# probabilists/zuko

Measured on AMD Instinct MI355X. Metric: log_prob samples/sec, NSF d=64 K=8 bins=8 batch=2^20, higher is better.
Workload: dtype f32; 1 GPU; NSF(features=64, context=0, transforms=8, bins=8, hidden=[256]*3) log_prob, batch=2^20 per GPU, x~N(0,1), seed-0 init; batch_per_gpu=1048576, global_batch=1048576, parallelism=batch-sharded x1, one RCCL all-reduce of the scalar NLL

## Files before the change

### zuko_amd/csrc/fused_ar_half_impl.h

```cpp
#pragma once
#include "fused_ar_split_impl.h"

#ifndef ARH_LOOK
#define ARH_LOOK 1
#endif
#ifndef ARH_RELU_INT
#define ARH_RELU_INT 0
#endif

namespace zk {

typedef _Float16 f16x8 __attribute__((ext_vector_type(8)));

struct ArhB {
  f16x8 h, l;
};

__device__ __forceinline__ void arh_scale(float amax, float& s, float& inv_s) {
  amax = fmaxf(amax, __shfl_xor(amax, 16, 64));
  amax = fmaxf(amax, __shfl_xor(amax, 32, 64));
  int e = __builtin_amdgcn_frexp_expf(amax);
  int ea = 15 - e;
  ea = ea > 90 ? 90 : (ea < -90 ? -90 : ea);
  s = __builtin_amdgcn_ldexpf(1.0f, ea);
  inv_s = __builtin_amdgcn_ldexpf(1.0f, -ea);
}

__device__ __forceinline__ void arh_split(const f32x4& lo, const f32x4& hi, float s, ArhB& b) {
  if (ARX_ABL == 6) {
    b.h = __builtin_bit_cast(f16x8, lo); b.l = __builtin_bit_cast(f16x8, hi);
    return;
  }
#pragma unroll
  for (int e = 0; e < 8; ++e) {
    const float v = (e < 4 ? lo[e] : hi[e - 4]) * s;
    const _Float16 h = (_Float16)v;
    const float r = v - (float)h;
    b.h[e] = h;
    b.l[e] = (_Float16)r;
  }
}

#define ARH_MFMA(A, B, C) C = __builtin_amdgcn_mfma_f32_16x16x32_f16(__builtin_bit_cast(f16x8, A), B, C, 0, 0, 0)
__device__ __forceinline__ void arh_block(const f32x4 (&a)[2], const ArhB& b, f32x4& c) {
  if (ARX_ABL == 2) {
    asm volatile("" ::"v"(a[0]), "v"(a[1]));
    return;
  }
  ARH_MFMA(a[1], b.h, c);
  ARH_MFMA(a[0], b.l, c);
  ARH_MFMA(a[0], b.h, c);
}

__device__ __forceinline__ void arh_touch(f32x4& v) { asm volatile("" : "+v"(v)); }
template <int N> __device__ __forceinline__ void arh_settle(f32x4& a0, f32x4& a1) { asm volatile("s_waitcnt lgkmcnt(%2)" : "+v"(a0), "+v"(a1) : "n"(N)); }
template <int N> __device__ __forceinline__ void arh_settle(f32x4& a0, f32x4& a1, f32x4& a2) { asm volatile("s_waitcnt lgkmcnt(%3)" : "+v"(a0), "+v"(a1), "+v"(a2) : "n"(N)); }

template <class S, int L, class Ring> __device__ __forceinline__ void arh_hidden(Ring& ring, const float* bias_q, const ArhB (&in)[S::TMAX / 2], f32x4 (&out)[S::TMAX], float d) {
  typedef ArxPat<S> P;
  constexpr int NB = S::NB[L], BASE = S::BASE[L], HTL = S::HT[L];
  ars_for<HTL>([&](auto t_) ARS_ALWAYS_INLINE {
    constexpr int t = t_;
    if constexpr (!P::tile_has_blocks(L, t)) out[t] = *reinterpret_cast<const f32x4*>(bias_q + t * 16);
  });
  if constexpr (NB > 0) {
    constexpr int LOOK = ARH_LOOK < NB ? ARH_LOOK : NB;
    f32x4 a[LOOK + 1][2];
    f32x4 bs;
    f32x4 acc;
    const unsigned bias_addr = arx_lds_addr(bias_q);
    ars_for<LOOK>([&](auto b_) ARS_ALWAYS_INLINE {
      constexpr int b = b_;
      ars_for<2>([&](auto p) ARS_ALWAYS_INLINE { a[b][p] = ring.template read<BASE + 2 * b + decltype(p)::value>(); });
    });
    ars_for<NB>([&](auto s_) ARS_ALWAYS_INLINE {
      constexpr int s = s_, ot = P::ot(L, s), ip = P::ip(L, s), cur = s % (LOOK + 1);
      constexpr bool first_of_tile = (s == 0 || P::ot(L, s - 1) != ot), last_of_tile = (s + 1 == NB || P::ot(L, s + 1) != ot);
      if constexpr (first_of_tile) acc = f32x4{0.f, 0.f, 0.f, 0.f};
      if constexpr (last_of_tile) bs = arx_lds_raw<ot * 64>(bias_addr);
      if constexpr (s + LOOK < NB) {
        constexpr int nx = (s + LOOK) % (LOOK + 1);
        ars_for<2>([&](auto p) ARS_ALWAYS_INLINE { a[nx][p] = ring.template read<BASE + 2 * (s + LOOK) + decltype(p)::value>(); });
      }
      constexpr int ahead = (s + LOOK < NB ? LOOK : NB - 1 - s);
      if constexpr (last_of_tile) arh_settle<(s + LOOK < NB ? 2 : 0)>(a[cur][0], a[cur][1], bs);
      else arh_settle<2 * ahead>(a[cur][0], a[cur][1]);
      if (ARX_FENCE) __builtin_amdgcn_sched_barrier(0);
      arh_block(a[cur], in[ip], acc);
      if (ARX_FENCE) __builtin_amdgcn_sched_barrier(0);
      if constexpr (last_of_tile) {
#pragma unroll
        for (int r = 0; r < 4; ++r) out[ot][r] = __builtin_fmaf(acc[r], d, bs[r]);
      }
    });
  }
}

template <class S, int L, class Ring> __device__ __forceinline__ void arh_hidden_stack(Ring& ring, const float* bias_lds, int q, ArhB (&in)[S::TMAX / 2], f32x4 (&out)[S::TMAX], const ArArgs& a,
                                                                                       float& inv_s) {
  if constexpr (L < S::NH) {
    arh_hidden<S, L>(ring, bias_lds + L * S::BIAS_STRIDE + 4 * q, in, out, a.wdescale[L] * inv_s);
    constexpr int HTL = S::HT[L];
    float amax = 0.f;
    if constexpr (S::ACT == 1) {
#pragma unroll
      for (int t = 0; t < HTL; ++t)
#pragma unroll
        for (int r = 0; r < 4; ++r) {
          if (ARH_RELU_INT) out[t][r] = __builtin_bit_cast(float, max(__builtin_bit_cast(int, out[t][r]), 0));
          else out[t][r] = out[t][r] < 0.f ? 0.f : out[t][r];
          amax = fmaxf(amax, out[t][r]);
        }
    } else {
      if constexpr (S::ACT != 0) {
#pragma unroll 1
        for (int rep = 0; rep < 1; ++rep) {
#pragma unroll
          for (int t = 0; t < HTL; ++t)
#pragma unroll
            for (int r = 0; r < 4; ++r) out[t][r] = act_f32(out[t][r], S::ACT);
        }
      }
#pragma unroll
      for (int t = 0; t < HTL; ++t)
#pragma unroll
        for (int r = 0; r < 4; ++r) amax = fmaxf(amax, fabsf(out[t][r]));
    }
    float s;
    arh_scale(amax, s, inv_s);
    const f32x4 zero = {0.f, 0.f, 0.f, 0.f};
#pragma unroll
    for (int p = 0; p < (HTL + 1) / 2; ++p) arh_split(out[2 * p], 2 * p + 1 < HTL ? out[2 * p + 1] : zero, s, in[p]);
    arh_hidden_stack<S, L + 1, Ring>(ring, bias_lds, q, in, out, a, inv_s);
  }
}

template <class S, typename Uni, bool DIAG = false> __global__ __launch_bounds__(64 * S::WAVES, S::OCC) void arh_kernel(ArArgs a) {
  typedef ArRingS<S::WAVES, S::CH, S::NR> Ring;
  static_assert(S::WAVES == 8 && S::NR == 3 && S::TMAX <= 16 && S::TMAX % 2 == 0 && S::OCC == 2, "two-part split kernels: widths <= 256, two wavefronts per SIMD");
  constexpr int NT = Uni::NT, FPL = Uni::FPL, TOTAL = Uni::TOTAL, WAVES = S::WAVES;
  constexpr int NG = S::NG;
  constexpr int NSTEP = S::GOFF[NG];
  constexpr bool XLDS = S::XLDS;
  constexpr bool FID_REGS = NG * FPL <= 32;
  constexpr int DT = (S::D + 15) / 16;
  const int tid = threadIdx.x;
  const int lane = tid & 63;
  const int wave = __builtin_amdgcn_readfirstlane(tid >> 6);
  const int j = lane & 15, q = lane >> 4;

  Ring ring;
  float* bias_lds = ars_lds + S::NR * S::CH * AR_TF;
  ring.lds = ars_lds; ring.stream = a.stream; ring.n_chunks = a.n_chunks; ring.wave = wave; ring.lane = lane;
  ring.load_chunk = 0; ring.load_slot = 0;
#pragma unroll
  for (int i = 0; i < S::NR - 1; ++i) ring.issue();
  ring.slot = S::NR - 1;
  ring.lds_off = (unsigned)(size_t)((__attribute__((address_space(3))) float*)ars_lds);
  ring.cur_off = ring.lds_off;

  for (int i = tid; i < a.bias_floats; i += 64 * WAVES) bias_lds[i] = a.bias[i];
  int* fmap_lds = reinterpret_cast<int*>(bias_lds + a.bias_floats);
  float* xr = reinterpret_cast<float*>(fmap_lds + 1024 + 256) + wave * 16 * a.xs + j * a.xs;
  for (int i = tid; i < NG * 4 * FPL; i += 64 * WAVES) fmap_lds[i] = a.featmap[i];
  __syncthreads();
  const float* bias_last = bias_lds + S::NH * S::BIAS_STRIDE;
  const unsigned bias_last_addr = arx_lds_addr(bias_last + 4 * q);
  int fids[FID_REGS ? NG * FPL : 1];
  if constexpr (FID_REGS) {
#pragma unroll
    for (int i = 0; i < NG; ++i)
#pragma unroll
      for (int fi = 0; fi < FPL; ++fi) fids[i * FPL + fi] = fmap_lds[(i * 4 + q) * FPL + fi];
  }

  for (int64_t tile = blockIdx.x; tile < a.n_tiles; tile += gridDim.x) {
    const int64_t n = tile * (16 * WAVES) + wave * 16 + j;
    const bool live = n < a.N;
    const int64_t nc = live ? n : a.N - 1;
    const float* xrow = a.x + nc * a.ldx;

    ArhB in[S::TMAX / 2];
    f32x4 out[S::TMAX];
    float poison = 0.f;
    float inv_s;
    {
      f32x4 xin[S::NIT + 1];
#pragma unroll
      for (int it = 0; it < S::NIT; ++it) {
        f32x4 v = {0.f, 0.f, 0.f, 0.f};
        if ((it + 1) * 16 <= S::DIN || it * 16 + 4 * q < S::DIN) v = *reinterpret_cast<const f32x4*>(xrow + it * 16 + 4 * q);
        xin[it] = v;
      }
      xin[S::NIT] = f32x4{0.f, 0.f, 0.f, 0.f};
      int bad = 0;
      float amax = 0.f;
#pragma unroll
      for (int it = 0; it < S::NIT; ++it)
#pragma unroll
        for (int r = 0; r < 4; ++r) {
          bad |= !(fabsf(xin[it][r]) < __builtin_inff());
          amax = fmaxf(amax, fabsf(xin[it][r]));
        }
      bad |= __shfl_xor(bad, 16, 64);
      bad |= __shfl_xor(bad, 32, 64);
      if (bad) poison = __builtin_nanf("");
      if constexpr (XLDS) {
#pragma unroll
        for (int it = 0; it < DT; ++it)
          if ((it + 1) * 16 <= S::D || it * 16 + 4 * q < S::D) *reinterpret_cast<f32x4*>(xr + it * 16 + 4 * q) = xin[it];
        asm volatile("" ::: "memory");
        __builtin_amdgcn_wave_barrier();
      }
      float s;
      arh_scale(amax, s, inv_s);
#pragma unroll
      for (int p = 0; p < (S::NIT + 1) / 2; ++p) arh_split(xin[2 * p], xin[2 * p + 1], s, in[p]);
    }

    arh_hidden_stack<S, 0, Ring>(ring, bias_lds, q, in, out, a, inv_s);

    const float dl = a.wdescale[S::NH] * inv_s;
    float lacc = 0.f;
    constexpr int NBL = NSTEP * NT;
    constexpr int LOOKL = ARH_LOOK < NBL ? ARH_LOOK : NBL;
    f32x4 w[LOOKL + 1][2];
    ars_for<LOOKL>([&](auto b_) ARS_ALWAYS_INLINE {
      constexpr int b = b_;
      ars_for<2>([&](auto p) ARS_ALWAYS_INLINE { w[b][p] = ring.template read<S::LAST_BASE + 2 * b + decltype(p)::value>(); });
    });
    ars_for<NG>([&](auto g_) ARS_ALWAYS_INLINE {
      constexpr int g = g_, ST0 = S::GOFF[g], GN = S::GOFF[g + 1] - S::GOFF[g];
      int fid[FPL];
      float xin[FPL];
#pragma unroll
      for (int fi = 0; fi < FPL; ++fi) {
        if constexpr (FID_REGS) fid[fi] = fids[g * FPL + fi];
        else fid[fi] = fmap_lds[(g * 4 + q) * FPL + fi];
        const int fc = fid[fi] < 0 ? 0 : fid[fi];
        if constexpr (XLDS) xin[fi] = xr[fc];
        else xin[fi] = xrow[fc];
      }
      f32x4 acc[NT], bs[NT];
      if constexpr (GN == 0) {
        const float* bg = bias_last + (g * NT) * 16 + 4 * q;
        ars_for<NT>([&](auto t) ARS_ALWAYS_INLINE { bs[t] = *reinterpret_cast<const f32x4*>(bg + t * 16); });
      }
      ars_for<NT>([&](auto t) ARS_ALWAYS_INLINE { acc[t] = f32x4{0.f, 0.f, 0.f, 0.f}; });
      ars_for<GN>([&](auto i_) ARS_ALWAYS_INLINE {
        constexpr int st = ST0 + decltype(i_)::value, ip = S::G_IP[st];
        ars_for<NT>([&](auto t_) ARS_ALWAYS_INLINE {
          constexpr int t = t_, blk = st * NT + t, cur = blk % (LOOKL + 1);
          constexpr bool last_of_group = (decltype(i_)::value == GN - 1 && t == NT - 1);
          if constexpr (last_of_group) {
            ars_for<NT>([&](auto u) ARS_ALWAYS_INLINE { bs[u] = arx_lds_raw<(g * NT + decltype(u)::value) * 64>(bias_last_addr); });
          }
          if constexpr (blk + LOOKL < NBL) {
            constexpr int nx = (blk + LOOKL) % (LOOKL + 1);
            ars_for<2>([&](auto p) ARS_ALWAYS_INLINE { w[nx][p] = ring.template read<S::LAST_BASE + 2 * (blk + LOOKL) + decltype(p)::value>(); });
          }
          constexpr int ahead = (blk + LOOKL < NBL ? LOOKL : NBL - 1 - blk);
          if constexpr (last_of_group) arh_settle<(blk + LOOKL < NBL ? 2 : 0)>(w[cur][0], w[cur][1]);
          else arh_settle<2 * ahead>(w[cur][0], w[cur][1]);
          if constexpr (last_of_group) {
#pragma unroll
            for (int u = 0; u < NT; ++u) arh_touch(bs[u]);
          }
          if (ARX_FENCE) __builtin_amdgcn_sched_barrier(0);
          arh_block(w[cur], in[ip], acc[t]);
          if (ARX_FENCE) __builtin_amdgcn_sched_barrier(0);
        });
      });
      float p[4 * NT];
      ars_for<NT>([&](auto t) ARS_ALWAYS_INLINE {
#pragma unroll
        for (int r = 0; r < 4; ++r) p[4 * t + r] = __builtin_fmaf(acc[t][r], dl, bs[t][r]);
      });
#pragma unroll
      for (int fi = 0; fi < FPL; ++fi) Uni::template poison<false>(p, fi * TOTAL, poison);
      auto ld = [&](int i) { return p[i]; };
#pragma unroll
      for (int fi = 0; fi < FPL; ++fi) {
        const int f = fid[fi];
        if (f >= 0) {
          float yv, lj;
          if (ARX_ABL == 3) {
            yv = p[fi * TOTAL] + xin[fi]; lj = p[fi * TOTAL + 1];
#pragma unroll
            for (int i = 2; i < TOTAL; ++i) lj += p[fi * TOTAL + i];
          } else if constexpr (DIAG) {
            int kb = 0;
            float ks[Uni::NKNOT];
            Uni::fwd(ld, fi * TOTAL, a, xin[fi], yv, lj, &kb, ks);
            if (live) {
              a.bin_out[n * S::D + f] = kb;
#pragma unroll
              for (int jj = 0; jj < Uni::NKNOT; ++jj) a.knots_out[(n * S::D + f) * Uni::NKNOT + jj] = ks[jj];
            }
          } else
          Uni::fwd(ld, fi * TOTAL, a, xin[fi], yv, lj);
          if constexpr (XLDS) xr[f] = yv;
          else if (live) a.y[n * a.ldy + f] = yv;
          lacc += lj;
        }
      }
    });
    if constexpr (XLDS) {
      asm volatile("" ::: "memory");
      __builtin_amdgcn_wave_barrier();
      if (live) {
#pragma unroll
        for (int it = 0; it < DT; ++it)
          if ((it + 1) * 16 <= S::D || it * 16 + 4 * q < S::D) *reinterpret_cast<f32x4*>(a.y + n * a.ldy + it * 16 + 4 * q) = *reinterpret_cast<const f32x4*>(xr + it * 16 + 4 * q);
      }
    }
    if (a.ladj) {
      lacc += __shfl_xor(lacc, 16, 64);
      lacc += __shfl_xor(lacc, 32, 64);
      if (live && q == 0) a.ladj[n] = a.accumulate ? a.ladj[n] + lacc : lacc;
    }
  }
  asm volatile("s_waitcnt vmcnt(0)" ::: "memory");
}

template <class S, typename Uni> static int arh_launch(const ArArgs* in, int abi, int args_bytes, int train, void* stream) {
  if (abi != ARS_ABI || args_bytes != (int)sizeof(ArArgs)) return ZK_EINVAL;
  ArArgs a = *in;
  if (train || a.D != S::D || a.DIN != S::DIN || a.L != S::NH + 1 || a.act != S::ACT || a.sched || a.NG != S::NG || a.n_chunks != S::NCHUNK || a.l1rev) return ZK_EINVAL;
  for (int l = 0; l <= S::NH; ++l)
    if (!(a.wdescale[l] > 0.f) || !(a.wdescale[l] < __builtin_inff())) return ZK_EINVAL;
  a.n_tiles = (a.N + 16 * S::WAVES - 1) / (16 * S::WAVES);
  a.xs = ((S::D + 3) / 4) * 4 + 4;
  const bool vec_ok = (S::D % 4 == 0) && (a.ldy % 4 == 0) && ((uintptr_t)a.y % 16 == 0);
  if (S::XLDS != 0 && !vec_ok) return ZK_EINVAL;
  a.xlds = S::XLDS;
  const int lds = (S::NR * S::CH * AR_TF + a.bias_floats + 1024 + 256 + (S::XLDS ? S::WAVES * 16 * a.xs : 0)) * (int)sizeof(float);
  if (lds > 160 * 1024) return ZK_EINVAL;
  const void* fn = nullptr;
  if ((a.bin_out != nullptr) != (a.knots_out != nullptr)) return ZK_EINVAL;
  if (a.bin_out) {
    if constexpr (Uni::NKNOT > 1) fn = (const void*)arh_kernel<S, Uni, true>;
  } else {
    fn = (const void*)arh_kernel<S, Uni, false>;
  }
  if (!fn) return ZK_EINVAL;
  hipError_t e = hipSuccess;
  {
    static std::mutex mu;
    static std::unordered_map<const void*, int> granted;
    std::lock_guard<std::mutex> lock(mu);
    int& g = granted[fn];
    if (g < lds) {
      e = hipFuncSetAttribute(fn, hipFuncAttributeMaxDynamicSharedMemorySize, lds);
// ... 13 lines not shown
```

### zuko_amd/static_ar.py

```python

from __future__ import annotations

import ctypes
import fcntl
import hashlib
import json
import math
import os
import shutil
import subprocess
import sys
import threading

import numpy as np

HERE = os.path.dirname(os.path.abspath(__file__))
CSRC = os.path.join(HERE, "csrc")
ARS_DIR = os.path.join(HERE, "lib", "ars")
ARS_ABI = 9
UNI_TYPES = {0: "zk::UniAffine", 1: "zk::UniRqs8", 2: "zk::UniRqs4", 3: "zk::UniRqs16", 4: "zk::UniCircRqs8", 5: "zk::UniSos3x5", 6: "zk::UniBern17"}
SPLIT_ONLY_KINDS = {3, 5, 6}
_HEADERS = ("fused_ar_static_impl.h", "fused_ar_split_impl.h", "zk_ar_common.h", "zk_univariate.h", "zk_univariate_bwd.h", "zk_common.h", "zk_half.h")


# ... 244 lines not shown
        GOFFP.append(len(G_IP))
    last_base = cursor
    cursor += 3 * len(blocks)
    n_chunks = -(-cursor // ch)
    pad_blocks = -(-(n_chunks * ch - cursor) // 3)
    blocks_of.append(blocks + [-np.ones((64, 8), dtype=np.int64)] * pad_blocks)
    stream_images = max(n_chunks * ch, cursor + 3 * pad_blocks)
    gathers = [np.stack(b).astype(np.int32).reshape(-1) if b else np.zeros(0, np.int32) for b in blocks_of]
    out = dict(t)
    for key in ("S_OTG", "S_IT", "S_MASK", "NS", "GOFF", "G_IT"):
        out.pop(key)
    nr = 2 if ch == 48 else 3
    per_cu = 2 if (waves == 4 and not wide) else 1
    xlds = int(t["D"] % 4 == 0 and (nr * ch * 256 + (t["BIAS_STRIDE"] * NH + t["NG"] * nt * 16) + 1024 + 256 + waves * 16 * (((t["D"] + 3) // 4) * 4 + 4)) * 4 * per_cu <= 160 * 1024)
    out.update({"split": 1, "TMAX": int(2 * -(-t["TMAX"] // 2)), "NB": NB, "B_OT": B_OT, "B_IP": B_IP, "BASE": BASE, "LAST_BASE": last_base, "GOFF": GOFFP, "G_IP": G_IP, "NCHUNK": n_chunks, "STREAM_IMAGES": stream_images,
                "WAVES": waves, "CH": ch, "NR": nr, "XLDS": xlds, "OCC": 1 if wide else 2})
    plan._split_cache = ((uni_kind, act, split_geometry()), (out, gathers))
    return out, gathers


def half_enabled() -> bool:
    from . import fused

    return split_enabled() and fused.matmul_precision() == "f16x2"


def half_tables(plan, uni_kind: int, act: int = 1):
    ts = split_tables(plan, uni_kind, act)
    if ts is None:
        return None
    t, gathers = ts
    if t["WAVES"] != 8 or t["NH"] > 3 or uni_kind in SPLIT_ONLY_KINDS or t["CH"] != 24:
        return None
    cached = getattr(plan, "_half_cache", None)
    if cached is not None and cached[0] == (uni_kind, act):
        return cached[1]
    ch, NH, nt = t["CH"], t["NH"], plan.layout.nt
    n_last = t["GOFF"][-1] * nt
    cursor = 2 * (sum(t["NB"]) + n_last)
    n_chunks = -(-cursor // ch)
    pad_blocks = -(-(n_chunks * ch - cursor) // 2)
    last = gathers[NH][: n_last * 512]
    g = [np.asarray(x) for x in gathers[:NH]] + [np.concatenate([last, -np.ones(pad_blocks * 512, dtype=np.int32)]).astype(np.int32)]
    out = {k: v for k, v in t.items() if k not in ("split", "TRAIN_OK")}
    out.update({"half": 1, "BASE": [2 * sum(t["NB"][:l]) for l in range(NH)], "LAST_BASE": 2 * sum(t["NB"]), "NCHUNK": n_chunks, "STREAM_IMAGES": max(n_chunks * ch, cursor + 2 * pad_blocks),
                "NR": 3, "TRAIN_OK": 0})
    plan._half_cache = ((uni_kind, act), (out, g))
    return out, g


def emit_half(t: dict) -> str:
    boff = [0]
    for n in t["NB"]:
        boff.append(boff[-1] + n)
    lines = [
        "// generated by zuko_amd/static_ar.py — do not edit",
        '#include "fused_ar_half_impl.h"',
        "namespace {",
        "struct Shape {",
        f"  static constexpr int D = {t['D']}, DIN = {t['DIN']}, NIT = {t['NIT']}, NH = {t['NH']}, TMAX = {t['TMAX']}, NG = {t['NG']}, NCHUNK = {t['NCHUNK']};",
        f"  static constexpr int BIAS_STRIDE = {t['BIAS_STRIDE']}, LAST_BASE = {t['LAST_BASE']}, WAVES = {t['WAVES']}, CH = {t['CH']}, NR = {t['NR']}, ACT = {t['ACT']}, OCC = {t['OCC']};",
        f"  static constexpr bool XLDS = {'true' if t['XLDS'] else 'false'};",
        _arr("HT", "int", t["HT"]), _arr("NB", "int", t["NB"]), _arr("BOFF", "int", boff), _arr("BASE", "int", t["BASE"]),
        _arr("B_OT", "unsigned char", t["B_OT"]), _arr("B_IP", "unsigned char", t["B_IP"]), _arr("GOFF", "int", t["GOFF"]), _arr("G_IP", "unsigned char", t["G_IP"]),
        "};",
        "}  // namespace",
        f'extern "C" int zk_ars_launch(const zk::ArArgs* a, int abi, int args_bytes, int train, void* stream) {{ return zk::arh_launch<Shape, {UNI_TYPES[t["uni"]]}>(a, abi, args_bytes, train, stream); }}',
        "",
    ]
    return "\n".join(lines)


def compile_half(t: dict, verbose: bool = False, out_dir: str | None = None) -> dict | None:
    stamp = _half_digest()
    sig = _digest({"half": t, "headers": stamp})
    meta = {"so": f"arh_{sig}.so", "core": "h" + _digest(t), "half": 1, "split": 2, "l0": [], "alt": None, "headers": stamp, "uni": t["uni"], "ACT": t["ACT"], "D": t["D"], "DIN": t["DIN"], "HT": t["HT"],
            "WAVES": t["WAVES"], "CH": t["CH"], "TRAIN_OK": 0, "XLDS": t["XLDS"], "NCHUNK": t["NCHUNK"]}
    so = _build_so(f"arh_{sig}", lambda: emit_half(t), meta, verbose, out_dir)
    if so is None:
        return None
    global _INDEX
# ... 539 lines not shown
                    cands.append(chain_tables_for(lins, full=True, packed={"uni": layout.kind, "featmap": pl.featmap, "nt": layout.nt, "fpl": layout.fpl, "total": layout.total}))
                for tg in cands:
                    if tg is not None and not any(c[0] == tg[0] for c in chains):
                        chains.append(tg)
        for pl in (pa, pd):
            ts = split_tables(pl, layout.kind, act)
            if ts is not None and not any(x == ts[0] for x in splits):
                splits.append(ts[0])
            th = half_tables(pl, layout.kind, act)
            if th is not None and not any(x == th[0] for x in halves):
                halves.append(th[0])
        if layout.kind in SPLIT_ONLY_KINDS:
            continue
        ta, td = tables(pa, layout.kind, act), tables(pd, layout.kind, act)
        if ta is None or td is None:
            raise RuntimeError(f"zuko_amd.static_ar: no static kernel for the prebuilt shape {entry}")
        (ca, la), (cdesc, ld) = _split(ta), _split(td)
        if ca == cdesc:
            work.append((ta, None if la == ld else ld))
        else:
            work += [(ta, None), (td, None)]
    prev = os.environ.get("ZUKO_AMD_SPLIT_GEOM")
    if prev is None:
        os.environ["ZUKO_AMD_SPLIT_GEOM"] = "4x16"
        try:
            kind, features, context, hidden, bins = PREBUILT[0][:5]
            for pl, layout, _ in _plans_for(kind, features, context, hidden, bins):
                pl._split_cache = None
                ts = split_tables(pl, layout.kind, 1)
                if ts is not None and not any(x == ts[0] for x in splits):
                    splits.append(ts[0])
        finally:
            del os.environ["ZUKO_AMD_SPLIT_GEOM"]
    with ThreadPoolExecutor(max_workers=jobs) as ex:
        metas = list(ex.map(lambda w: compile_kernel(w[0], w[1], verbose, ARS_DIR), work))
        kerns = list(ex.map(lambda tg: chain_kernel(tg[0], True, verbose, ARS_DIR), chains))
        xmetas = list(ex.map(lambda t: compile_split(t, verbose, ARS_DIR), splits))
        hmetas = list(ex.map(lambda t: compile_half(t, verbose, ARS_DIR), halves))
    if any(m is None for m in metas + xmetas + hmetas) or any(k is None for k in kerns):
        raise RuntimeError("zuko_amd.static_ar: a prebuilt static kernel failed to compile")
    return [m["so"] for m in metas + xmetas + hmetas] + [os.path.basename(k.so) for k in kerns]


if __name__ == "__main__":
    sys.path.insert(0, os.path.dirname(HERE))
    import zuko_amd.static_ar as me

    print("\n".join(me.prebuild()))
```

### zuko_amd/csrc/zk_ar_common.h

```cpp
#pragma once
#include "zk_univariate.h"

namespace zk {

typedef float f32x4 __attribute__((ext_vector_type(4)));

#define AR_TF 256
#define AR_WAVES 8
#define AR_T 16
#define ARS_ABI 9

struct ArArgs {
  int64_t N;
  int D, DIN;
  const float* x; int64_t ldx;
  float* y; int64_t ldy;
  const float* yin; int64_t ldyin;
  float* ladj; int accumulate;
  const float* stream;
  const float* bias;
  const uint32_t* skip;
  const int32_t* featmap;
  int L, NG, n_chunks, act, bias_floats, dbg;
  const int* sched;
  int n_sched;
  int olim[8];
  int g0, g1;
  int xlds;
  int xs;
  float bound, ls;
  RqsLeanConst lc;
  int64_t n_tiles;
  int32_t* bin_out;
  float* knots_out;
  int l1rev;
  float* act_out[3];
  float* phi_out;
  int64_t ldphi;
  const float* gate[3];
  const float* phi_in;
  float* gphi_out;
  int64_t ldpin;
  const float* gy; int64_t ldgy;
// ... 13 lines not shown
    case 4: return v / (1.f + expf(-v));
    case 5: return 0.5f * v * (1.f + erff(v * 0.70710678118654752440f));
    case 6: return 1.f / (1.f + expf(-v));
    case 7: return v > 0.f ? v : 0.01f * v;
    default: return v;
  }
}


struct UniAffine {
  static constexpr int TOTAL = 2, FPL = 2, NT = 1;
  template <bool INV> static __device__ __forceinline__ void poison(float* p, int base, float nan_or_zero) {
    p[base + 0] += nan_or_zero;
    p[base + 1] += nan_or_zero;
  }
  static constexpr int NKNOT = 1;
  template <typename P, typename A> static __device__ __forceinline__ void fwd(const P& p, int base, const A& a, float x, float& y, float& lj, int* k = nullptr, float* ks = nullptr) {
    affine_fwd<float, MathFast>(p(base + 0), p(base + 1), a.ls, x, y, lj);
  }
  template <typename P, typename A> static __device__ __forceinline__ float inv(const P& p, int base, const A& a, float y) {
    return affine_inv<float, MathFast>(p(base + 0), p(base + 1), a.ls, y);
  }
};

template <int K, bool CIRC> struct UniRqs {
  static constexpr int TOTAL = 3 * K - 1, FPL = 1, NT = (TOTAL + 3) / 4;
  static __device__ __forceinline__ float shift(float v, float bound) {
    const float period = 2.f * bound;
    float r = fmodf(v, period);
    r = (r < 0.f) ? r + period : r;
    return r - bound;
  }
  template <bool INV> static __device__ __forceinline__ void poison(float* p, int base, float nan_or_zero) {
#pragma unroll
    for (int j = 0; j < K; ++j) p[base + (INV ? K : 0) + j] += nan_or_zero;
  }
  static constexpr int NKNOT = K + 1;
  template <typename P, typename A> static __device__ __forceinline__ void fwd(const P& p, int base, const A& a, float x, float& y, float& lj, int* k = nullptr, float* ks = nullptr) {
    int kk;
    rqs_lean<K, false>([&](int j) { return p(base + j); }, [&](int j) { return p(base + K + j); }, [&](int j) { return p(base + 2 * K + j); }, a.lc,
                       CIRC ? shift(x, a.bound) : x, y, lj, kk, ks);
    if (k) *k = kk;
  }
  template <typename P, typename A> static __device__ __forceinline__ float inv(const P& p, int base, const A& a, float y) {
    float x, lj;
    rqs_lean<K, true>([&](int j) { return p(base + j); }, [&](int j) { return p(base + K + j); }, [&](int j) { return p(base + 2 * K + j); }, a.lc, y, x, lj);
    return CIRC ? shift(x, a.bound) : x;
  }
};
template <int P, int L1> struct UniSos {
  static constexpr int TOTAL = P * L1 + 1, FPL = 1, NT = (TOTAL + 3) / 4, NKNOT = 1;
  template <bool INV> static __device__ __forceinline__ void poison(float* p, int base, float nan_or_zero) {
    p[base] += nan_or_zero;
    p[base + P * L1] += nan_or_zero;
  }
  template <typename Pa, typename A> static __device__ __forceinline__ void fwd(const Pa& p, int base, const A& a, float x, float& y, float& lj, int* k = nullptr, float* ks = nullptr) {
    auto ld = [&](int j) { return p(base + j); };
    y = sos_f_static<float, P, L1>(a.sos, ld, x) + p(base + P * L1);
    lj = t_log(sos_g_static<float, P, L1>(a.sos, ld, x));
  }
};
template <int NC> struct UniBernBounded {
  static constexpr int TOTAL = NC - 5, FPL = 1, NT = (TOTAL + 3) / 4, NKNOT = 1;
  template <bool INV> static __device__ __forceinline__ void poison(float* p, int base, float nan_or_zero) { p[base] += nan_or_zero; }
  template <typename Pa, typename A> static __device__ __forceinline__ void fwd(const Pa& p, int base, const A& a, float x, float& y, float& lj, int* k = nullptr, float* ks = nullptr) {
    float th[NC];
    bern_theta_bounded<float, NC>([&](int j) { return p(base + j); }, a.bound, th);
    const BernTails<float> t = bern_tails<float, NC>(th, true, a.bound, a.eps);
// ... 14 lines not shown
```

### zuko_amd/fused.py

```python

from __future__ import annotations

from dataclasses import dataclass

import ctypes
import math
import os

import numpy as np
import torch
from torch import Tensor

TILE = 16
CHUNK = 24
GROUP_HIDDEN = 4
MAX_WIDTH = 256
MAX_WIDTH_WIDE = 512


@dataclass
class UniLayout:

    kind: int
    total: int
# ... 336 lines not shown
_precision = None


def matmul_precision() -> str:
    global _precision
    if _precision is None:
        _precision = _PRECISIONS.get(os.environ.get("ZUKO_AMD_MATMUL", "f16x2").lower(), "f16x2")
    return _precision


def set_matmul_precision(mode: str) -> None:
    global _precision
    if mode.lower() not in _PRECISIONS:
        raise ValueError(f"zuko_amd.set_matmul_precision: unknown mode '{mode}' (one of {sorted(_PRECISIONS)})")
    _precision = _PRECISIONS[mode.lower()]


HALF_SPREAD_LOG2 = 14
HALF_SMALL_FRACTION = 0.01
HALF_ROW_LOG2 = 12
HALF_MIN_LOG2, HALF_MAX_LOG2 = -20, 40


def half_scales(linears):
    stats = []
    for m in linears:
        w = m.weight.detach()
        a = (w * m.mask).abs() if getattr(m, "mask", None) is not None else w.abs()
        big = a.amax()
        nz = a > 0
        small = (nz & (a < big * 2.0 ** -HALF_SPREAD_LOG2)).sum() / nz.sum().clamp_min(1)
        rowmax = a.amax(dim=1)
        minrow = torch.where(rowmax > 0, rowmax, big).amin()
        stats.append(torch.stack([big.float(), small.float(), minrow.float()]))
    out = []
    for big, small, minrow in torch.stack(stats).tolist():
        if big == 0.0:
            out.append((True, 0))
            continue
        ok = math.isfinite(big) and 2.0 ** HALF_MIN_LOG2 <= big <= 2.0 ** HALF_MAX_LOG2 and small <= HALF_SMALL_FRACTION and minrow >= big * 2.0 ** -HALF_ROW_LOG2
        out.append((bool(ok), 15 - math.frexp(big)[1] if math.isfinite(big) else 0))
    return out


def chunk_of(variant: int = 0) -> int:
    return CHUNK


def default_variant() -> int:
    return 0


class FusedAR:

    def __init__(self, plan: ArPlan, device: torch.device, act: int, bound: float, slope: float, variant: int = 0) -> None:
        self.plan = plan
        self.variant = variant
        self.device = device
        self.act = act
        self.bound = bound
        self.slope = slope
        self.skip = torch.from_numpy(plan.skip.view(np.int32).copy()).to(device)
        self.featmap = torch.from_numpy(plan.featmap.copy()).to(device)
        self.gather = [torch.from_numpy(g).to(device) for g in plan.gather]
        self.bias_gather = [torch.from_numpy(g).to(device) for g in plan.bias_gather]
        self.stream = torch.empty(plan.n_blocks * 256, dtype=torch.float32, device=device)
        self.bias_floats = plan.bias_off[-1] + len(plan.bias_gather[-1])
        self.bias = torch.empty(self.bias_floats, dtype=torch.float32, device=device)
        self._stamp = None
        self._fine_stamp = None
        self.generic_ok = plan.max_width <= MAX_WIDTH and plan.layout.kind <= 4
        self.eps = 1e-6
        self._gl = None
# ... 280 lines not shown
```

Before: 70.82 million samples/s.

## Use fma_mix f16 split, asm ReLU, packed descale, and selectable half ring geometry

```diff
diff --git a/zuko_amd/csrc/fused_ar_half_impl.h b/zuko_amd/csrc/fused_ar_half_impl.h
--- a/zuko_amd/csrc/fused_ar_half_impl.h
+++ b/zuko_amd/csrc/fused_ar_half_impl.h
@@ -26,19 +26,123 @@
   inv_s = __builtin_amdgcn_ldexpf(1.0f, -ea);
 }
 
+#ifndef ARH_SPLIT_FORM
+#define ARH_SPLIT_FORM 4
+#endif
+typedef _Float16 f16x2 __attribute__((ext_vector_type(2)));
+typedef float f32x2 __attribute__((ext_vector_type(2)));
+
 __device__ __forceinline__ void arh_split(const f32x4& lo, const f32x4& hi, float s, ArhB& b) {
   if (ARX_ABL == 6) {
     b.h = __builtin_bit_cast(f16x8, lo); b.l = __builtin_bit_cast(f16x8, hi);
     return;
   }
-#pragma unroll
-  for (int e = 0; e < 8; ++e) {
-    const float v = (e < 4 ? lo[e] : hi[e - 4]) * s;
-    const _Float16 h = (_Float16)v;
-    const float r = v - (float)h;
-    b.h[e] = h;
-    b.l[e] = (_Float16)r;
-  }
+  if constexpr (ARH_SPLIT_FORM == 0) {
+#pragma unroll
+    for (int e = 0; e < 8; ++e) {
+      const float v = (e < 4 ? lo[e] : hi[e - 4]) * s;
+      const _Float16 h = (_Float16)v;
+      const float r = v - (float)h;
+      b.h[e] = h;
+      b.l[e] = (_Float16)r;
+    }
+  } else {
+    typedef unsigned u32x4 __attribute__((ext_vector_type(4)));
+    u32x4 hp, lp;
+#pragma unroll
+    for (int p = 0; p < 4; ++p) {
+      const float x0 = p < 2 ? lo[2 * p] : hi[2 * p - 4], x1 = p < 2 ? lo[2 * p + 1] : hi[2 * p - 3];
+      if constexpr (ARH_SPLIT_FORM == 1) {
+        const f32x2 v = f32x2{x0, x1} * f32x2{s, s};
+        const f16x2 h = __builtin_convertvector(v, f16x2);
+        const f32x2 r = v - __builtin_convertvector(h, f32x2);
+        hp[p] = __builtin_bit_cast(unsigned, h);
+        lp[p] = __builtin_bit_cast(unsigned, __builtin_convertvector(r, f16x2));
+      } else if constexpr (ARH_SPLIT_FORM == 2) {
+        const float v0 = x0 * s, v1 = x1 * s;
+        const f16x2 h = __builtin_convertvector(f32x2{v0, v1}, f16x2);
+        const float r0 = v0 - (float)h[0], r1 = v1 - (float)h[1];
+        hp[p] = __builtin_bit_cast(unsigned, h);
+        lp[p] = __builtin_bit_cast(unsigned, __builtin_convertvector(f32x2{r0, r1}, f16x2));
+      } else if constexpr (ARH_SPLIT_FORM == 3) {
+        const float v0 = x0 * s, v1 = x1 * s;
+        unsigned h, l;
+        asm("v_cvt_pk_f16_f32 %0, %1, %2" : "=v"(h) : "v"(v0), "v"(v1));
+        asm("v_fma_mixlo_f16 %0, %1, 1.0, -%2 op_sel_hi:[0,0,1]" : "=v"(l) : "v"(v0), "v"(h));
+        asm("v_fma_mixhi_f16 %0, %1, 1.0, -%2 op_sel:[0,0,1] op_sel_hi:[0,0,1]" : "+v"(l) : "v"(v1), "v"(h));
+        hp[p] = h;
+        lp[p] = l;
+      } else {
+        unsigned h, l;
+        asm("v_fma_mixlo_f16 %0, %1, %2, 0" : "=v"(h) : "v"(x0), "v"(s));
+        asm("v_fma_mixhi_f16 %0, %1, %2, 0" : "+v"(h) : "v"(x1), "v"(s));
+        asm("v_fma_mixlo_f16 %0, %1, %2, -%3 op_sel_hi:[0,0,1]" : "=v"(l) : "v"(x0), "v"(s), "v"(h));
+        asm("v_fma_mixhi_f16 %0, %1, %2, -%3 op_sel:[0,0,1] op_sel_hi:[0,0,1]" : "+v"(l) : "v"(x1), "v"(s), "v"(h));
+        hp[p] = h;
+        lp[p] = l;
+      }
+    }
+    b.h = __builtin_bit_cast(f16x8, hp);
+    b.l = __builtin_bit_cast(f16x8, lp);
+  }
+}
+
+#ifndef ARH_RELU_FORM
+#define ARH_RELU_FORM 1
+#endif
+__device__ __forceinline__ void arh_relu(f32x4& v) {
+  if constexpr (ARH_RELU_FORM == 0) {
+#pragma unroll
+    for (int r = 0; r < 4; ++r) v[r] = v[r] < 0.f ? 0.f : v[r];
+  } else if constexpr (ARH_RELU_FORM == 2) {
+#pragma unroll
+    for (int r = 0; r < 4; ++r) {
+      float x = v[r];
+      asm("v_max_f32 %0, 0, %0" : "+v"(x));
+      v[r] = x;
+    }
+  } else if constexpr (ARH_RELU_FORM == 3) {
+#pragma unroll
+    for (int r = 0; r < 4; ++r) {
+      float x = v[r];
+      int t;
+      asm("v_add_i32 %1, %0, %2 clamp\n\t"
+          "v_ashrrev_i32 %1, 31, %1\n\t"
+          "v_bfi_b32 %0, %1, 0, %0"
+          : "+v"(x), "=&v"(t) : "s"(0x7fffff));
+      v[r] = x;
+    }
+  } else {
+    unsigned long long m0, m1, m2, m3;
+    float a = v[0], b = v[1], c = v[2], d = v[3];
+    asm("s_nop 0\n\t"
+        "v_cmp_ngt_f32_e64 %4, 0, %0\n\t"
+        "v_cmp_ngt_f32_e64 %5, 0, %1\n\t"
+        "v_cmp_ngt_f32_e64 %6, 0, %2\n\t"
+        "v_cmp_ngt_f32_e64 %7, 0, %3\n\t"
+        "v_cndmask_b32_e64 %0, 0, %0, %4\n\t"
+        "v_cndmask_b32_e64 %1, 0, %1, %5\n\t"
+        "v_cndmask_b32_e64 %2, 0, %2, %6\n\t"
+        "v_cndmask_b32_e64 %3, 0, %3, %7"
+        : "+v"(a), "+v"(b), "+v"(c), "+v"(d), "=&s"(m0), "=&s"(m1), "=&s"(m2), "=&s"(m3));
+    v = f32x4{a, b, c, d};
+  }
+}
+
+#ifndef ARH_DESCALE_PK
+#define ARH_DESCALE_PK 1
+#endif
+__device__ __forceinline__ f32x4 arh_descale(const f32x4& acc, float d, const f32x4& bs) {
+  f32x4 o;
+  if constexpr (ARH_DESCALE_PK) {
+    const f32x2 dd = {d, d};
+    const f32x2 lo = __builtin_elementwise_fma(f32x2{acc[0], acc[1]}, dd, f32x2{bs[0], bs[1]}), hi = __builtin_elementwise_fma(f32x2{acc[2], acc[3]}, dd, f32x2{bs[2], bs[3]});
+    o = f32x4{lo[0], lo[1], hi[0], hi[1]};
+  } else {
+#pragma unroll
+    for (int r = 0; r < 4; ++r) o[r] = __builtin_fmaf(acc[r], d, bs[r]);
+  }
+  return o;
 }
 
 #define ARH_MFMA(A, B, C) C = __builtin_amdgcn_mfma_f32_16x16x32_f16(__builtin_bit_cast(f16x8, A), B, C, 0, 0, 0)
@@ -88,10 +192,7 @@
       if (ARX_FENCE) __builtin_amdgcn_sched_barrier(0);
       arh_block(a[cur], in[ip], acc);
       if (ARX_FENCE) __builtin_amdgcn_sched_barrier(0);
-      if constexpr (last_of_tile) {
-#pragma unroll
-        for (int r = 0; r < 4; ++r) out[ot][r] = __builtin_fmaf(acc[r], d, bs[r]);
-      }
+      if constexpr (last_of_tile) out[ot] = arh_descale(acc, d, bs);
     });
   }
 }
@@ -104,13 +205,16 @@
     float amax = 0.f;
     if constexpr (S::ACT == 1) {
 #pragma unroll
-      for (int t = 0; t < HTL; ++t)
-#pragma unroll
-        for (int r = 0; r < 4; ++r) {
-          if (ARH_RELU_INT) out[t][r] = __builtin_bit_cast(float, max(__builtin_bit_cast(int, out[t][r]), 0));
-          else out[t][r] = out[t][r] < 0.f ? 0.f : out[t][r];
-          amax = fmaxf(amax, out[t][r]);
+      for (int t = 0; t < HTL; ++t) {
+        if (ARH_RELU_INT) {
+#pragma unroll
+          for (int r = 0; r < 4; ++r) out[t][r] = __builtin_bit_cast(float, max(__builtin_bit_cast(int, out[t][r]), 0));
+        } else {
+          arh_relu(out[t]);
         }
+#pragma unroll
+        for (int r = 0; r < 4; ++r) amax = fmaxf(amax, out[t][r]);
+      }
     } else {
       if constexpr (S::ACT != 0) {
 #pragma unroll 1
@@ -137,7 +241,7 @@
 
 template <class S, typename Uni, bool DIAG = false> __global__ __launch_bounds__(64 * S::WAVES, S::OCC) void arh_kernel(ArArgs a) {
   typedef ArRingS<S::WAVES, S::CH, S::NR> Ring;
-  static_assert(S::WAVES == 8 && S::NR == 3 && S::TMAX <= 16 && S::TMAX % 2 == 0 && S::OCC == 2, "two-part split kernels: widths <= 256, two wavefronts per SIMD");
+  static_assert(S::WAVES == 8 && (S::NR == 2 || S::NR == 3) && S::TMAX <= 16 && S::TMAX % 2 == 0 && S::OCC == 2, "two-part split kernels: widths <= 256, two wavefronts per SIMD");
   constexpr int NT = Uni::NT, FPL = Uni::FPL, TOTAL = Uni::TOTAL, WAVES = S::WAVES;
   constexpr int NG = S::NG;
   constexpr int NSTEP = S::GOFF[NG];
diff --git a/zuko_amd/static_ar.py b/zuko_amd/static_ar.py
--- a/zuko_amd/static_ar.py
+++ b/zuko_amd/static_ar.py
@@ -300,10 +300,11 @@
     t, gathers = ts
     if t["WAVES"] != 8 or t["NH"] > 3 or uni_kind in SPLIT_ONLY_KINDS or t["CH"] != 24:
         return None
+    geom = half_geometry(t, plan.bias_off[-1] + len(plan.bias_gather[-1]))
     cached = getattr(plan, "_half_cache", None)
-    if cached is not None and cached[0] == (uni_kind, act):
+    if cached is not None and cached[0] == (uni_kind, act, geom):
         return cached[1]
-    ch, NH, nt = t["CH"], t["NH"], plan.layout.nt
+    (ch, nr), NH, nt = geom, t["NH"], plan.layout.nt
     n_last = t["GOFF"][-1] * nt
     cursor = 2 * (sum(t["NB"]) + n_last)
     n_chunks = -(-cursor // ch)
@@ -312,9 +313,35 @@
     g = [np.asarray(x) for x in gathers[:NH]] + [np.concatenate([last, -np.ones(pad_blocks * 512, dtype=np.int32)]).astype(np.int32)]
     out = {k: v for k, v in t.items() if k not in ("split", "TRAIN_OK")}
     out.update({"half": 1, "BASE": [2 * sum(t["NB"][:l]) for l in range(NH)], "LAST_BASE": 2 * sum(t["NB"]), "NCHUNK": n_chunks, "STREAM_IMAGES": max(n_chunks * ch, cursor + 2 * pad_blocks),
-                "NR": 3, "TRAIN_OK": 0})
-    plan._half_cache = ((uni_kind, act), (out, g))
+                "CH": ch, "NR": nr, "TRAIN_OK": 0})
+    plan._half_cache = ((uni_kind, act, geom), (out, g))
     return out, g
+
+
+HALF_GEOMS = ((24, 3), (32, 3), (48, 2))
+HALF_GEOM_PREFERENCE = ((24, 3),)
+LDS_BYTES = 160 * 1024
+
+
+def half_lds_bytes(t: dict, bias_floats: int, ch: int, nr: int) -> int:
+    xs = ((t["D"] + 3) // 4) * 4 + 4
+    return (nr * ch * 256 + bias_floats + 1024 + 256 + (t["WAVES"] * 16 * xs if t["XLDS"] else 0)) * 4
+
+
+def half_geometry(t: dict, bias_floats: int) -> tuple:
+    env = os.environ.get("ZUKO_AMD_HALF_GEOM")
+    cands = HALF_GEOM_PREFERENCE
+    if env:
+        try:
+            c, n = (int(v) for v in env.split("x"))
+            if (c, n) in HALF_GEOMS:
+                cands = ((c, n),)
+        except ValueError:
+            pass
+    for c, n in cands:
+        if half_lds_bytes(t, bias_floats, c, n) <= LDS_BYTES:
+            return (c, n)
+    return (24, 3)
 
 
 def emit_half(t: dict) -> str:
@@ -920,6 +947,18 @@
                     splits.append(ts[0])
         finally:
             del os.environ["ZUKO_AMD_SPLIT_GEOM"]
+    prev = os.environ.get("ZUKO_AMD_HALF_GEOM")
+    if prev is None:
+        try:
+            for ch, nr in HALF_GEOMS:
+                os.environ["ZUKO_AMD_HALF_GEOM"] = f"{ch}x{nr}"
+                for entry in PREBUILT[:2]:
+                    for pl, layout, _ in _plans_for(*entry[:5]):
+                        th = half_tables(pl, layout.kind, 1)
+                        if th is not None and not any(x == th[0] for x in halves):
+                            halves.append(th[0])
+        finally:
+            del os.environ["ZUKO_AMD_HALF_GEOM"]
     with ThreadPoolExecutor(max_workers=jobs) as ex:
         metas = list(ex.map(lambda w: compile_kernel(w[0], w[1], verbose, ARS_DIR), work))
         kerns = list(ex.map(lambda tg: chain_kernel(tg[0], True, verbose, ARS_DIR), chains))
```

New measurement: 71.35 million samples/s, median of 6. Within noise of the previous version (+0.7%).

## Prefetch next tile inputs, pin split/relu epilogue asm, trim poison work

Applied to the files above, without the earlier changes.

```diff
diff --git a/zuko_amd/csrc/fused_ar_half_impl.h b/zuko_amd/csrc/fused_ar_half_impl.h
--- a/zuko_amd/csrc/fused_ar_half_impl.h
+++ b/zuko_amd/csrc/fused_ar_half_impl.h
@@ -6,6 +6,15 @@
 #endif
 #ifndef ARH_RELU_INT
 #define ARH_RELU_INT 0
+#endif
+#ifndef ARH_EPI_PINNED
+#define ARH_EPI_PINNED 1
+#endif
+#ifndef ARH_DESCALE_PK
+#define ARH_DESCALE_PK 1
+#endif
+#ifndef ARH_PREFETCH
+#define ARH_PREFETCH 1
 #endif
 
 namespace zk {
@@ -16,7 +25,7 @@
   f16x8 h, l;
 };
 
-__device__ __forceinline__ void arh_scale(float amax, float& s, float& inv_s) {
+__device__ __forceinline__ void arh_scale(float& amax, float& s, float& inv_s) {
   amax = fmaxf(amax, __shfl_xor(amax, 16, 64));
   amax = fmaxf(amax, __shfl_xor(amax, 32, 64));
   int e = __builtin_amdgcn_frexp_expf(amax);
@@ -26,11 +35,30 @@
   inv_s = __builtin_amdgcn_ldexpf(1.0f, -ea);
 }
 
+#define ARH_AMAX_OVERFLOW (65520.f * 0x1p90f)
+
+typedef unsigned arh_u32x4 __attribute__((ext_vector_type(4)));
+typedef float arh_f32x2 __attribute__((ext_vector_type(2)));
+
 __device__ __forceinline__ void arh_split(const f32x4& lo, const f32x4& hi, float s, ArhB& b) {
   if (ARX_ABL == 6) {
     b.h = __builtin_bit_cast(f16x8, lo); b.l = __builtin_bit_cast(f16x8, hi);
     return;
   }
+#if ARH_EPI_PINNED
+  const float nz = -0.f;
+  arh_u32x4 h, l;
+#pragma unroll
+  for (int e = 0; e < 4; ++e) asm("v_fma_mixlo_f16 %0, %1, %2, %3" : "=v"(h[e]) : "v"(e < 2 ? lo[2 * e] : hi[2 * e - 4]), "v"(s), "s"(nz));
+#pragma unroll
+  for (int e = 0; e < 4; ++e) asm("v_fma_mixhi_f16 %0, %1, %2, %3" : "+v"(h[e]) : "v"(e < 2 ? lo[2 * e + 1] : hi[2 * e - 3]), "v"(s), "s"(nz));
+#pragma unroll
+  for (int e = 0; e < 4; ++e) asm("v_fma_mixlo_f16 %0, %1, %2, -%3 op_sel:[0,0,0] op_sel_hi:[0,0,1]" : "=v"(l[e]) : "v"(e < 2 ? lo[2 * e] : hi[2 * e - 4]), "v"(s), "v"(h[e]));
+#pragma unroll
+  for (int e = 0; e < 4; ++e) asm("v_fma_mixhi_f16 %0, %1, %2, -%3 op_sel:[0,0,1] op_sel_hi:[0,0,1]" : "+v"(l[e]) : "v"(e < 2 ? lo[2 * e + 1] : hi[2 * e - 3]), "v"(s), "v"(h[e]));
+  b.h = __builtin_bit_cast(f16x8, h); b.l = __builtin_bit_cast(f16x8, l);
+  return;
+#endif
 #pragma unroll
   for (int e = 0; e < 8; ++e) {
     const float v = (e < 4 ? lo[e] : hi[e - 4]) * s;
@@ -55,6 +83,33 @@
 __device__ __forceinline__ void arh_touch(f32x4& v) { asm volatile("" : "+v"(v)); }
 template <int N> __device__ __forceinline__ void arh_settle(f32x4& a0, f32x4& a1) { asm volatile("s_waitcnt lgkmcnt(%2)" : "+v"(a0), "+v"(a1) : "n"(N)); }
 template <int N> __device__ __forceinline__ void arh_settle(f32x4& a0, f32x4& a1, f32x4& a2) { asm volatile("s_waitcnt lgkmcnt(%3)" : "+v"(a0), "+v"(a1), "+v"(a2) : "n"(N)); }
+
+template <int WAVES, int CH, int NR> struct ArhRing : ArRingS<WAVES, CH, NR> {
+  typedef ArRingS<WAVES, CH, NR> B;
+  template <int XV> __device__ __forceinline__ void advance_x() {
+    asm volatile("s_waitcnt vmcnt(%0) lgkmcnt(0)" ::"n"((NR - 2) * B::PER + XV) : "memory");
+    if (ARX_ABL != 4) __builtin_amdgcn_s_barrier();
+    asm volatile("" ::: "memory");
+    this->issue();
+    this->slot = (this->slot + 1 == NR) ? 0 : this->slot + 1;
+    this->cur_off = this->lds_off + (unsigned)(this->slot * CH * AR_TF * 4 + this->lane * 16);
+  }
+  template <int S, int XV = 0> __device__ __forceinline__ f32x4 read() {
+    if constexpr (XV != 0 && S % CH == 0) {
+      advance_x<XV>();
+      f32x4 v;
+      if (ARX_ABL == 5) {
+        asm volatile("v_mov_b32 %0, %1" : "=v"(v[0]) : "v"(this->cur_off));
+        v[1] = v[2] = v[3] = v[0];
+        return v;
+      }
+      asm volatile("ds_read_b128 %0, %1 offset:%2" : "=v"(v) : "v"(this->cur_off), "n"((S % CH) * AR_TF * 4));
+      return v;
+    } else {
+      return B::template read<S>();
+    }
+  }
+};
 
 template <class S, int L, class Ring> __device__ __forceinline__ void arh_hidden(Ring& ring, const float* bias_q, const ArhB (&in)[S::TMAX / 2], f32x4 (&out)[S::TMAX], float d) {
   typedef ArxPat<S> P;
@@ -89,20 +144,37 @@
       arh_block(a[cur], in[ip], acc);
       if (ARX_FENCE) __builtin_amdgcn_sched_barrier(0);
       if constexpr (last_of_tile) {
-#pragma unroll
-        for (int r = 0; r < 4; ++r) out[ot][r] = __builtin_fmaf(acc[r], d, bs[r]);
+        if (ARH_DESCALE_PK) {
+#pragma unroll
+          for (int r = 0; r < 4; r += 2) {
+            const arh_f32x2 o = __builtin_elementwise_fma(arh_f32x2{acc[r], acc[r + 1]}, arh_f32x2{d, d}, arh_f32x2{bs[r], bs[r + 1]});
+            out[ot][r] = o[0]; out[ot][r + 1] = o[1];
+          }
+        } else {
+#pragma unroll
+          for (int r = 0; r < 4; ++r) out[ot][r] = __builtin_fmaf(acc[r], d, bs[r]);
+        }
       }
     });
   }
 }
 
 template <class S, int L, class Ring> __device__ __forceinline__ void arh_hidden_stack(Ring& ring, const float* bias_lds, int q, ArhB (&in)[S::TMAX / 2], f32x4 (&out)[S::TMAX], const ArArgs& a,
-                                                                                       float& inv_s) {
+                                                                                       float& inv_s, float& poison) {
   if constexpr (L < S::NH) {
     arh_hidden<S, L>(ring, bias_lds + L * S::BIAS_STRIDE + 4 * q, in, out, a.wdescale[L] * inv_s);
     constexpr int HTL = S::HT[L];
     float amax = 0.f;
-    if constexpr (S::ACT == 1) {
+    if constexpr (S::ACT == 1 && ARH_EPI_PINNED) {
+#pragma unroll
+      for (int t = 0; t < HTL; ++t)
+#pragma unroll
+        for (int r = 0; r < 4; r += 2) {
+          asm("v_max_f32 %0, 0, %0" : "+v"(out[t][r]));
+          asm("v_max_f32 %0, 0, %0" : "+v"(out[t][r + 1]));
+          asm("v_max3_f32 %0, %0, %1, %2" : "+v"(amax) : "v"(out[t][r]), "v"(out[t][r + 1]));
+        }
+    } else if constexpr (S::ACT == 1) {
 #pragma unroll
       for (int t = 0; t < HTL; ++t)
 #pragma unroll
@@ -128,15 +200,18 @@
     }
     float s;
     arh_scale(amax, s, inv_s);
+    if constexpr (S::ACT == 1 && ARH_EPI_PINNED) {
+      if (!(amax < ARH_AMAX_OVERFLOW)) poison = __builtin_nanf("");
+    }
     const f32x4 zero = {0.f, 0.f, 0.f, 0.f};
 #pragma unroll
     for (int p = 0; p < (HTL + 1) / 2; ++p) arh_split(out[2 * p], 2 * p + 1 < HTL ? out[2 * p + 1] : zero, s, in[p]);
-    arh_hidden_stack<S, L + 1, Ring>(ring, bias_lds, q, in, out, a, inv_s);
+    arh_hidden_stack<S, L + 1, Ring>(ring, bias_lds, q, in, out, a, inv_s, poison);
   }
 }
 
 template <class S, typename Uni, bool DIAG = false> __global__ __launch_bounds__(64 * S::WAVES, S::OCC) void arh_kernel(ArArgs a) {
-  typedef ArRingS<S::WAVES, S::CH, S::NR> Ring;
+  typedef ArhRing<S::WAVES, S::CH, S::NR> Ring;
   static_assert(S::WAVES == 8 && S::NR == 3 && S::TMAX <= 16 && S::TMAX % 2 == 0 && S::OCC == 2, "two-part split kernels: widths <= 256, two wavefronts per SIMD");
   constexpr int NT = Uni::NT, FPL = Uni::FPL, TOTAL = Uni::TOTAL, WAVES = S::WAVES;
   constexpr int NG = S::NG;
@@ -159,6 +234,18 @@
   ring.lds_off = (unsigned)(size_t)((__attribute__((address_space(3))) float*)ars_lds);
   ring.cur_off = ring.lds_off;
 
+  auto x_request = [&](int64_t tile, f32x4 (&xv)[S::NIT]) ARS_ALWAYS_INLINE {
+    const int64_t n = tile * (16 * WAVES) + wave * 16 + j;
+    const float* row = a.x + (n < a.N ? n : a.N - 1) * a.ldx;
+#pragma unroll
+    for (int it = 0; it < S::NIT; ++it) {
+      const int col = it * 16 + 4 * q;
+      xv[it] = *reinterpret_cast<const f32x4*>(row + ((it + 1) * 16 <= S::DIN || col < S::DIN ? col : S::DIN - 4));
+    }
+  };
+  f32x4 xnext[S::NIT];
+  if (ARH_PREFETCH) x_request(blockIdx.x, xnext);
+
   for (int i = tid; i < a.bias_floats; i += 64 * WAVES) bias_lds[i] = a.bias[i];
   int* fmap_lds = reinterpret_cast<int*>(bias_lds + a.bias_floats);
   float* xr = reinterpret_cast<float*>(fmap_lds + 1024 + 256) + wave * 16 * a.xs + j * a.xs;
@@ -189,7 +276,11 @@
 #pragma unroll
       for (int it = 0; it < S::NIT; ++it) {
         f32x4 v = {0.f, 0.f, 0.f, 0.f};
-        if ((it + 1) * 16 <= S::DIN || it * 16 + 4 * q < S::DIN) v = *reinterpret_cast<const f32x4*>(xrow + it * 16 + 4 * q);
+        if (ARH_PREFETCH) {
+          if ((it + 1) * 16 <= S::DIN || it * 16 + 4 * q < S::DIN) v = xnext[it];
+        } else {
+          if ((it + 1) * 16 <= S::DIN || it * 16 + 4 * q < S::DIN) v = *reinterpret_cast<const f32x4*>(xrow + it * 16 + 4 * q);
+        }
         xin[it] = v;
       }
       xin[S::NIT] = f32x4{0.f, 0.f, 0.f, 0.f};
@@ -214,20 +305,33 @@
       }
       float s;
       arh_scale(amax, s, inv_s);
+      if constexpr (S::ACT == 1 && ARH_EPI_PINNED) {
+        if (!(amax < ARH_AMAX_OVERFLOW)) poison = __builtin_nanf("");
+      }
 #pragma unroll
       for (int p = 0; p < (S::NIT + 1) / 2; ++p) arh_split(xin[2 * p], xin[2 * p + 1], s, in[p]);
     }
 
-    arh_hidden_stack<S, 0, Ring>(ring, bias_lds, q, in, out, a, inv_s);
+    float ladj_in = 0.f;
+    if (ARH_PREFETCH && a.ladj && a.accumulate && live && q == 0) ladj_in = a.ladj[n];
+
+    arh_hidden_stack<S, 0, Ring>(ring, bias_lds, q, in, out, a, inv_s, poison);
 
     const float dl = a.wdescale[S::NH] * inv_s;
     float lacc = 0.f;
     constexpr int NBL = NSTEP * NT;
     constexpr int LOOKL = ARH_LOOK < NBL ? ARH_LOOK : NBL;
     f32x4 w[LOOKL + 1][2];
+    constexpr int XPOS = ARH_PREFETCH ? (S::LAST_BASE + S::CH - 1) / S::CH * S::CH : -1;
+    if (ARH_PREFETCH) {
+      asm volatile("" ::: "memory");
+      x_request(tile + gridDim.x < a.n_tiles ? tile + gridDim.x : tile, xnext);
+      asm volatile("" ::: "memory");
+    }
+#define ARH_READ_LAST(POS) ring.template read<(POS), ((POS) == XPOS ? S::NIT : 0)>()
     ars_for<LOOKL>([&](auto b_) ARS_ALWAYS_INLINE {
       constexpr int b = b_;
-      ars_for<2>([&](auto p) ARS_ALWAYS_INLINE { w[b][p] = ring.template read<S::LAST_BASE + 2 * b + decltype(p)::value>(); });
+      ars_for<2>([&](auto p) ARS_ALWAYS_INLINE { w[b][p] = ARH_READ_LAST(S::LAST_BASE + 2 * b + decltype(p)::value); });
     });
     ars_for<NG>([&](auto g_) ARS_ALWAYS_INLINE {
       constexpr int g = g_, ST0 = S::GOFF[g], GN = S::GOFF[g + 1] - S::GOFF[g];
@@ -257,7 +361,7 @@
           }
           if constexpr (blk + LOOKL < NBL) {
             constexpr int nx = (blk + LOOKL) % (LOOKL + 1);
-            ars_for<2>([&](auto p) ARS_ALWAYS_INLINE { w[nx][p] = ring.template read<S::LAST_BASE + 2 * (blk + LOOKL) + decltype(p)::value>(); });
+            ars_for<2>([&](auto p) ARS_ALWAYS_INLINE { w[nx][p] = ARH_READ_LAST(S::LAST_BASE + 2 * (blk + LOOKL) + decltype(p)::value); });
           }
           constexpr int ahead = (blk + LOOKL < NBL ? LOOKL : NBL - 1 - blk);
           if constexpr (last_of_group) arh_settle<(blk + LOOKL < NBL ? 2 : 0)>(w[cur][0], w[cur][1]);
@@ -274,7 +378,10 @@
       float p[4 * NT];
       ars_for<NT>([&](auto t) ARS_ALWAYS_INLINE {
 #pragma unroll
-        for (int r = 0; r < 4; ++r) p[4 * t + r] = __builtin_fmaf(acc[t][r], dl, bs[t][r]);
+        for (int r = 0; r < 4; ++r) {
+          p[4 * t + r] = __builtin_fmaf(acc[t][r], dl, bs[t][r]);
+          if (ARH_POISON_ONE) asm("" : "+v"(p[4 * t + r]));
+        }
       });
 #pragma unroll
       for (int fi = 0; fi < FPL; ++fi) Uni::template poison<false>(p, fi * TOTAL, poison);
@@ -305,6 +412,15 @@
         }
       }
     });
+#undef ARH_READ_LAST
+    auto ladj_out = [&]() ARS_ALWAYS_INLINE {
+      if (a.ladj) {
+        lacc += __shfl_xor(lacc, 16, 64);
+        lacc += __shfl_xor(lacc, 32, 64);
+        if (live && q == 0) a.ladj[n] = a.accumulate ? (ARH_PREFETCH ? ladj_in : a.ladj[n]) + lacc : lacc;
+      }
+    };
+    if (ARH_PREFETCH) ladj_out();
     if constexpr (XLDS) {
       asm volatile("" ::: "memory");
       __builtin_amdgcn_wave_barrier();
@@ -314,11 +430,7 @@
           if ((it + 1) * 16 <= S::D || it * 16 + 4 * q < S::D) *reinterpret_cast<f32x4*>(a.y + n * a.ldy + it * 16 + 4 * q) = *reinterpret_cast<const f32x4*>(xr + it * 16 + 4 * q);
       }
     }
-    if (a.ladj) {
-      lacc += __shfl_xor(lacc, 16, 64);
-      lacc += __shfl_xor(lacc, 32, 64);
-      if (live && q == 0) a.ladj[n] = a.accumulate ? a.ladj[n] + lacc : lacc;
-    }
+    if (!ARH_PREFETCH) ladj_out();
   }
   asm volatile("s_waitcnt vmcnt(0)" ::: "memory");
 }
diff --git a/zuko_amd/csrc/zk_ar_common.h b/zuko_amd/csrc/zk_ar_common.h
--- a/zuko_amd/csrc/zk_ar_common.h
+++ b/zuko_amd/csrc/zk_ar_common.h
@@ -9,6 +9,9 @@
 #define AR_WAVES 8
 #define AR_T 16
 #define ARS_ABI 9
+#ifndef ARH_POISON_ONE
+#define ARH_POISON_ONE 1
+#endif
 
 struct ArArgs {
   int64_t N;
@@ -88,8 +91,12 @@
     return r - bound;
   }
   template <bool INV> static __device__ __forceinline__ void poison(float* p, int base, float nan_or_zero) {
+#if ARH_POISON_ONE
+    p[base + (INV ? K : 0)] += nan_or_zero;
+#else
 #pragma unroll
     for (int j = 0; j < K; ++j) p[base + (INV ? K : 0) + j] += nan_or_zero;
+#endif
   }
   static constexpr int NKNOT = K + 1;
   template <typename P, typename A> static __device__ __forceinline__ void fwd(const P& p, int base, const A& a, float x, float& y, float& lj, int* k = nullptr, float* ks = nullptr) {
diff --git a/zuko_amd/fused.py b/zuko_amd/fused.py
--- a/zuko_amd/fused.py
+++ b/zuko_amd/fused.py
@@ -392,13 +392,15 @@
         small = (nz & (a < big * 2.0 ** -HALF_SPREAD_LOG2)).sum() / nz.sum().clamp_min(1)
         rowmax = a.amax(dim=1)
         minrow = torch.where(rowmax > 0, rowmax, big).amin()
-        stats.append(torch.stack([big.float(), small.float(), minrow.float()]))
+        bias = getattr(m, "bias", None)
+        bfin = torch.isfinite(bias.detach()).all() if bias is not None else torch.ones((), dtype=torch.bool, device=w.device)
+        stats.append(torch.stack([big.float(), small.float(), minrow.float(), bfin.float()]))
     out = []
-    for big, small, minrow in torch.stack(stats).tolist():
+    for big, small, minrow, bfin in torch.stack(stats).tolist():
         if big == 0.0:
-            out.append((True, 0))
+            out.append((bfin == 1.0, 0))
             continue
-        ok = math.isfinite(big) and 2.0 ** HALF_MIN_LOG2 <= big <= 2.0 ** HALF_MAX_LOG2 and small <= HALF_SMALL_FRACTION and minrow >= big * 2.0 ** -HALF_ROW_LOG2
+        ok = bfin == 1.0 and math.isfinite(big) and 2.0 ** HALF_MIN_LOG2 <= big <= 2.0 ** HALF_MAX_LOG2 and small <= HALF_SMALL_FRACTION and minrow >= big * 2.0 ** -HALF_ROW_LOG2
         out.append((bool(ok), 15 - math.frexp(big)[1] if math.isfinite(big) else 0))
     return out
 
```

After: 73.30 million samples/s before, 75.28 million samples/s after (median of 6 runs). +2.7%, better.
